# piotrprzybyszdev/Path-Tracing

Hardware: AMD Instinct MI355X
Metric: Msamples/s (paths*spp/s) at 1920x1080, 8spp, depth 8 (higher is better)
Workload: dtype f32; 1 GPU; chess_like (procedural stand-in for BASELINE configs[1] 'Khronos ABeautifulGame'), 1920x1080, 8 spp, depth 8; triangles=1999000, frames_in_flight=8, parallelism=pixel-tile shard x1, backend=wavefront, tile=32

## Files before the change

### path-tracing_amd/csrc/pt_render_host.hpp

```cpp
#pragma once

#include <type_traits>

template <typename F> static void withMode(int mode, F &&f)
{
    if (mode == 2) f(std::integral_constant<int, 2>());
    else if (mode == 1) f(std::integral_constant<int, 1>());
    else f(std::integral_constant<int, 0>());
}
template <typename F> static void withFlag(bool flag, F &&f)
{
    if (flag) f(std::true_type());
    else f(std::false_type());
}

static int ensureSlots(PtxRenderer *r, size_t slots)
{
    PathState &ps = r->paths;
    const size_t want = std::max(slots, ps.slotRad.n);
    const int mode = kernelMode(r);
    if (mode >= 1)
        HIP_TRY(r, ps.diffs.alloc(3 * want));
    if (mode == 2)
    {
// ... 55 lines not shown
    uint32_t tailBelow;
    uint32_t sortShade;
    Wavefront wf, wfAux;
};

static int counterErrors(PtxRenderer *r)
{
    const uint32_t *h = r->hostCounters;
    if (h[C_OVERFLOW])
        return fail(r, PTX_ERROR_DEVICE, "ptx_render: traversal stack overflow (tree deeper than %d levels)", kLdsStack + kGlobalSpill);
    if (h[C_OVERFLOW + 1])
        return fail(r, PTX_ERROR_DEVICE, "ptx_render: %u paths never produced a finite sample in %u attempts", h[C_OVERFLOW + 1], kMaxSampleRetries);
    return PTX_OK;
}

static int fetchCounters(PtxRenderer *r)
{
    HIP_TRY(r, hipMemcpyAsync(r->hostCounters, r->counters.p, C_COUNT * sizeof(uint32_t), hipMemcpyDeviceToHost, r->stream));
    HIP_TRY(r, hipStreamSynchronize(r->stream));
    return counterErrors(r);
}

static void launchAccumulate(PtxRenderer *r, const LaunchParams &p)
{
    k_accumulate<<<gridFor((size_t)p.slotsPerFrame * p.framesPerWave), kBlock, 0, r->stream>>>(p, r->paths.slotRad.p, accumTarget(r), nullptr, r->boundShard ? 1u : 0u);
}

static void launchTail(PtxRenderer *r, const RenderPlan &pl, int queue, uint32_t paths, BounceCtl ctl)
{
    const dim3 grid(gridFor(paths, kBlock, kMaxPersistentThreads / kBlock));
    withMode(pl.mode, [&](auto M) { k_tail<decltype(M)::value><<<grid, kBlock, 0, r->auxStream>>>(pl.p, pl.sv, pl.sc, pl.wfAux, queue, ctl); });
}

static int enqueueBounce(PtxRenderer *r, const RenderPlan &pl, uint32_t b, int qin, uint32_t est, int tail, bool fresh)
{
    hipStream_t S = r->stream, X = r->auxStream;
    PtxRenderer::BounceEvents &ev = r->bounceEvents[(b - 1) % r->bounceEvents.size()];
    const BounceCtl ctl = { b, 0u };
    const int qout = qin ^ 1, parity = (int)(b & 1u);
    k_prologue<<<1, 1, 0, S>>>(pl.wf, qin, ctl);
    HIP_TRY(r, hipEventRecord(ev.t0, S));
    withFlag(pl.mode == 2, [&](auto ALPHA) {
        const dim3 grid(traceGridFor(est, r->residentClosest[decltype(ALPHA)::value]));
        if (fresh)
            k_trace_closest<FirstBounce, decltype(ALPHA)::value><<<grid, kBlock, 0, S>>>(pl.sc, pl.wf, r->launchParams.p, pl.p.numSlots);
        else
            k_trace_closest<decltype(ALPHA)::value><<<grid, kBlock, 0, S>>>(pl.sc, pl.wf, qin, ctl);
    });
    HIP_TRY(r, hipEventRecord(ev.t1, S));
    if (b > 1)
        HIP_TRY(r, hipStreamWaitEvent(S, r->bounceEvents[(b - 2) % r->bounceEvents.size()].x2, 0));
    const uint32_t shadeGrid = gridFor((est + kShadeItems - 1) / kShadeItems);
    withFlag(pl.mode >= 1, [&](auto TEXTURED) {
        constexpr bool TEX = decltype(TEXTURED)::value;
        if (pl.sortShade && fresh)
            k_shade_sorted<FirstBounce, TEX><<<shadeGrid, kBlock, 0, S>>>(pl.p, pl.sv, pl.wf, qin, ctl);
        else if (pl.sortShade)
            k_shade_sorted<TEX><<<shadeGrid, kBlock, 0, S>>>(pl.p, pl.sv, pl.wf, qin, ctl);
        else if (fresh)
            k_shade<FirstBounce, TEX><<<shadeGrid, kBlock, 0, S>>>(pl.p, pl.sv, pl.wf, qin, ctl);
        else
            k_shade<TEX><<<shadeGrid, kBlock, 0, S>>>(pl.p, pl.sv, pl.wf, qin, ctl);
    });
    HIP_TRY(r, hipEventRecord(ev.t2, S));
    HIP_TRY(r, hipStreamWaitEvent(X, ev.t2, 0));
    HIP_TRY(r, hipEventRecord(ev.x0, X));
    withFlag(pl.mode == 2, [&](auto ALPHA) {
        k_trace_shadow<decltype(ALPHA)::value><<<traceGridFor(est, r->residentShadow[decltype(ALPHA)::value]), kBlock, 0, X>>>(pl.p, pl.sc, pl.wfAux, qout, parity);
    });
    k_apply_shadow<<<gridFor(est, kBlock, 4096u), kBlock, 0, X>>>(pl.p, pl.wfAux, parity);
    HIP_TRY(r, hipEventRecord(ev.x1, X));
    if (tail)
    {
        const uint32_t room = tail == 2 ? 4u * pl.tailBelow : pl.tailBelow;
        launchTail(r, pl, qout, est < room ? est : room, { b, tail == 2 ? 0xffffffffu : pl.tailBelow });
    }
    HIP_TRY(r, hipEventRecord(ev.x2, X));
    return PTX_OK;
}

static void hintedSchedule(const uint32_t *hint, uint32_t bounces, uint32_t tailBelow, uint32_t upperBound, std::vector<BounceStep> &steps)
{
    uint32_t last = bounces;
    if (tailBelow)
        for (uint32_t b = 1; b < bounces && b < (uint32_t)kMaxTimedBounces; b++)
            if (hint[b + 1] <= tailBelow) { last = b; break; }
    steps.clear();
    for (uint32_t b = 1; b <= last; b++)
    {
        uint32_t est = upperBound;
        if (b > 1 && b <= (uint32_t)kMaxTimedBounces)
            est = (uint32_t)std::min<uint64_t>((uint64_t)hint[b] + hint[b] / 4 + 4096, upperBound);
        steps.push_back({ b, est, (b == last && last < bounces) ? 2 : 0 });
    }
}

static int enqueueRound(PtxRenderer *r, const RenderPlan &pl, uint32_t upperBound, const uint32_t *hint, bool fresh)
{
    uint32_t last = 0;
    int qin = 0;
    if (hint)
    {
        hintedSchedule(hint, pl.bounces, pl.tailBelow, upperBound, r->hint.steps);
        for (const BounceStep &s : r->hint.steps)
        {
            if (const int rc = enqueueBounce(r, pl, s.bounce, qin, s.est, s.tail, fresh && s.bounce == 1u))
                return rc;
            last = s.bounce;
            qin ^= 1;
        }
    }
    else
    {
        uint32_t est = upperBound;
        for (uint32_t b = 1; b <= pl.bounces; b++)
        {
            if (const int rc = enqueueBounce(r, pl, b, qin, est, 0, fresh && b == 1u))
                return rc;
            last = b;
            qin ^= 1;
            if (const int rc = fetchCounters(r))
                return rc;
            est = r->hostCounters[qin ? C_ACTIVE1 : C_ACTIVE0];
            if (est == 0u)
                break;
            if (b < pl.bounces && est <= pl.tailBelow)
            {
                launchTail(r, pl, qin, est, { b, 0xffffffffu });
                HIP_TRY(r, hipEventRecord(r->bounceEvents[(b - 1) % r->bounceEvents.size()].x2, r->auxStream));
                break;
            }
        }
    }
    if (last)
        HIP_TRY(r, hipStreamWaitEvent(r->stream, r->bounceEvents[(last - 1) % r->bounceEvents.size()].x2, 0));
    HIP_TRY(r, hipGetLastError());
    return PTX_OK;
}

static int collectRender(PtxRenderer *r)
{
    if (r->pending.kind == PendingLaunch::kNone)
        return PTX_OK;
    const PendingLaunch pd = r->pending;
    r->pending = PendingLaunch();
    HIP_TRY(r, hipEventSynchronize(r->evB));
    if (const int rc = counterErrors(r))
        return rc;
    const uint32_t *h = r->hostCounters;
    r->stats.shadowRays = h[C_HITS];
// ... 5 lines not shown
    }
    unsigned long long waveSegments = 0;
    std::memcpy(&waveSegments, &h[C_WAVE_SEGMENTS], sizeof(waveSegments));
    waveSegments -= pd.deadSlots;
    r->stats.segments = waveSegments + h[C_SEGMENTS];
    r->stats.tracedRays = waveSegments;
    r->stats.retries = h[C_RETRIES];
    const uint32_t timed = pd.bounces < (uint32_t)kMaxTimedBounces ? pd.bounces : (uint32_t)kMaxTimedBounces;
    const uint32_t tailPaths = h[C_TAIL_PATHS], tailBounce = h[C_TAIL_PATHS + 1];
    for (uint32_t b = 1; b <= timed; b++)
    {
        const PtxRenderer::BounceEvents &ev = r->bounceEvents[b - 1];
        const uint32_t active = h[C_BOUNCE_ACTIVE + b];
        const bool ran = active != 0u && !(tailPaths && b > tailBounce);
        if (!ran)
            continue;
        float closestMs = 0.0f, shadeMs = 0.0f, shadowMs = 0.0f, tailMs = 0.0f;
        (void)hipEventElapsedTime(&closestMs, ev.t0, ev.t1);
        (void)hipEventElapsedTime(&shadeMs, ev.t1, ev.t2);
        (void)hipEventElapsedTime(&shadowMs, ev.x0, ev.x1);
        r->stats.lastTraceMs += closestMs;
        r->stats.lastShadeMs += shadeMs;
        r->stats.lastShadowMs += shadowMs;
        r->stats.traceLaunches += 2;
        if (tailPaths && tailBounce == b)
        {
            (void)hipEventElapsedTime(&tailMs, ev.x1, ev.x2);
            r->stats.lastTailMs += tailMs;
        }
        if (pd.verbose)
        {
            fprintf(stderr, "[ptx] bounce %u: %u rays closest %.3f ms (%.2f Grays/s) | shade (incl. wait for the previous shadow kernel) %.3f ms | shadow %.3f ms\n",
                    b, active, closestMs, active / closestMs / 1e6, shadeMs, shadowMs);
            if (tailMs > 0.0f)
                fprintf(stderr, "[ptx] tail: %u paths, %u segments, %.3f ms\n", tailPaths, h[C_SEGMENTS], tailMs);
        }
    }
    if (pd.verbose && h[C_RETRIES])
        fprintf(stderr, "[ptx] %u NaN / Inf sample restarts\n", h[C_RETRIES]);
    r->hint.active.assign(h + C_BOUNCE_ACTIVE, h + C_BOUNCE_ACTIVE + kMaxTimedBounces + 1);
    if (tailPaths && tailBounce + 1 <= (uint32_t)kMaxTimedBounces)
        r->hint.active[tailBounce + 1] = tailPaths;
    r->hint.slots = pd.slots; r->hint.bounces = pd.bounces; r->hint.epoch = pd.epoch;
    if (tailPaths > pd.tailBelow)
        r->hint.forget();
    return PTX_OK;
}

static int beginLaunch(PtxRenderer *r, const PtxLightsUbo *lights, const LaunchParams &p, uint64_t slots)
{
    HIP_TRY(r, hipSetDevice(r->device));
    if (const int rc = collectRender(r))
        return rc;
    if (const int rc = waitForCommits(r))
        return rc;
    if (slots > 0x7fffffffull)
        return fail(r, PTX_ERROR_INVALID_ARGUMENT, "ptx_render: too many path slots in one batch");
    if (const int rc = slots ? ensureSlots(r, (size_t)slots) : PTX_OK)
        return rc;
    k_upload_lights<<<1, 256, 0, r->stream>>>(*lights, p, r->lights.p, r->launchParams.p);
    HIP_TRY(r, hipMemsetAsync(r->counters.p, 0, C_COUNT * sizeof(uint32_t), r->stream));
    r->stats.pathSamples = r->stats.segments = r->stats.shadowRays = r->stats.retries = r->stats.tracedRays = 0;
    r->stats.traceLaunches = 0;
    r->stats.lastTraceMs = r->stats.lastShadeMs = r->stats.lastShadowMs = r->stats.lastTailMs = 0.0;
    HIP_TRY(r, hipEventRecord(r->evA, r->stream));
    return PTX_OK;
}

static int endLaunch(PtxRenderer *r, const PendingLaunch &pd)
{
    HIP_TRY(r, hipMemcpyAsync(r->hostCounters, r->counters.p, C_COUNT * sizeof(uint32_t), hipMemcpyDeviceToHost, r->stream));
    HIP_TRY(r, hipEventRecord(r->evB, r->stream));
    HIP_TRY(r, hipGetLastError());
// ... 43 lines not shown
    {
        if (const int rc = fetchCounters(r))
            return rc;
        const uint32_t restarts = r->hostCounters[C_RESTART];
        if (!restarts)
            return PTX_OK;
        if (round > maxRounds)
            return fail(r, PTX_ERROR_DEVICE, "ptx_render: %u paths still active after %llu rounds", restarts, (unsigned long long)maxRounds);
        k_restart<<<gridFor(restarts), kBlock, 0, r->stream>>>(pl.p, pl.wf, restarts);
        HIP_TRY(r, hipMemcpyAsync(pl.wf.queue[0], pl.wf.restartQueue, (size_t)restarts * sizeof(uint32_t), hipMemcpyDeviceToDevice, r->stream));
        HIP_TRY(r, hipMemsetAsync(&r->counters.p[C_RESTART], 0, sizeof(uint32_t), r->stream));
        HIP_TRY(r, hipMemsetD32Async(reinterpret_cast<hipDeviceptr_t>(&r->counters.p[C_ACTIVE0]), (int)restarts, 1, r->stream));
        if (const int rc = enqueueRound(r, pl, restarts, nullptr, false))
            return rc;
    }
}

static int renderWavefront(PtxRenderer *r, RenderPlan &pl, uint32_t sampleCount)
{
    const LaunchParams &p = pl.p;
    if (const int rc = ensureRenderResources(r, pl.bounces))
        return rc;
    pl.sortShade = r->env.shadeSort >= 0 ? (uint32_t)r->env.shadeSort : (sceneOf(r)->scene.mixedMaterialTypes || sceneOf(r)->scene.mixedTextured) ? 1u : 0u;
    pl.tailBelow = r->env.tailThreshold >= 0 ? (uint32_t)r->env.tailThreshold : 75000u;
    pl.wf = r->paths.view(pl.mode, r->counters.p, r->spill.p);
    pl.wfAux = r->paths.view(pl.mode, r->counters.p, r->spillAux.p);
    const bool canonical = sampleCount == 1;
    const uint64_t epoch = sceneOf(r)->sceneEpoch;
    const uint32_t *hint = canonical && r->hint.matches(p.numSlots, pl.bounces, epoch) ? r->hint.active.data() : nullptr;
    const bool fresh = r->env.firstBounce;
    if (!fresh)
        k_generate<<<gridFor(p.numSlots), kBlock, 0, r->stream>>>(p, pl.wf);
    HIP_TRY(r, hipMemsetD32Async(reinterpret_cast<hipDeviceptr_t>(&r->counters.p[C_ACTIVE0]), (int)p.numSlots, 1, r->stream));
    if (const int rc = enqueueRound(r, pl, p.numSlots, hint, fresh))
        return rc;
    if (canonical)
        finishCanonical(r, pl);
    else if (const int rc = runSampleRounds(r, pl, sampleCount))
        return rc;
    launchAccumulate(r, p);
    return endLaunch(r, { PendingLaunch::kWavefront, pl.bounces, pl.tailBelow, canonical ? p.numSlots : 0u, p.numSlots - p.ownedPixels * p.frames, epoch, r->env.verbose });
}

static int renderImpl(PtxRenderer *r, const PtxRaygenUniformData *uniform, const PtxLightsUbo *lights, uint32_t firstFrame, uint32_t frames)
{
    if (!r || !uniform || !lights)
        return fail(r, PTX_ERROR_INVALID_ARGUMENT, "ptx_render: null argument");
    if (!sceneUsable(r) || !imagePtr(r))
        return fail(r, PTX_ERROR_NOT_READY, "ptx_render: need ptx_scene_upload (or ptx_share_scene), ptx_build_accel and ptx_resize first");
    if (uniform->SampleCount == 0 || uniform->SampleCount > 0xffffu || uniform->BounceCount > 0xffffu || frames == 0)
        return fail(r, PTX_ERROR_INVALID_ARGUMENT, "ptx_render: SampleCount must be in [1, 65535], BounceCount <= 65535");
    if (lights->LightCount > PTX_MAX_LIGHT_COUNT)
        return fail(r, PTX_ERROR_INVALID_ARGUMENT, "ptx_render: LightCount %u exceeds MaxLightCount", lights->LightCount);
    RenderPlan pl;
    pl.p = makeParams(r, uniform, firstFrame, frames);
    if (const int rc = beginLaunch(r, lights, pl.p, (uint64_t)pl.p.slotsPerFrame * frames))
        return rc;
    if (pl.p.numSlots == 0)
    {
        HIP_TRY(r, hipEventRecord(r->evB, r->stream));
        return PTX_OK;
    }
    pl.sv = makeSceneView(r); pl.sc = makeTraceScene(r);
    pl.mode = kernelMode(r); pl.bounces = uniform->BounceCount;
    if (r->backend == PTX_BACKEND_MEGAKERNEL)
        return renderMegakernel(r, pl);
    if (pl.bounces == 0)
        return renderZeroBounces(r, pl.p, uniform->SampleCount);
    return renderWavefront(r, pl, uniform->SampleCount);
}

static int renderDebug(PtxRenderer *r, const PtxRaygenUniformData *uniform, const PtxLightsUbo *lights, const PtxDebugViewDesc *view)
{
    if (!r || !uniform || !lights || !view)
// ... 35 lines not shown
```

### path-tracing_amd/csrc/pt_runtime.hpp

```cpp
#pragma once

#include <algorithm>
#include <atomic>
#include <cstdarg>
#include <cstdio>
#include <cstdlib>
#include <cstring>
#include <memory>
#include <string>
#include <vector>

#include "pt_aux_kernels.hpp"
#include "pt_bvh_build.hpp"
#include "pt_debug_view.hpp"
#include "pt_denoise.hpp"
#include "pt_post.hpp"
#include "pt_present.hpp"


template <typename T> struct DevBuf
{
    T *p = nullptr;
    size_t n = 0;
    DevBuf() = default;
// ... 33 lines not shown
    uint32_t plocRadius = kPlocRadius;
    float plocShape = kPlocShape;
    bool mortonCubic = false;
    uint32_t collapse = 1;
    uint32_t reinsertPasses = 2;
    uint32_t reinsertFinal = 32;
    float splitBudget = 0.0f;
    uint32_t layout = 0;
};

struct EnvSwitches
{
    uint32_t cuPartition = 0;
    bool singleStream = false;
    bool verbose = false;
    bool karrasBuilder = false;
    bool plocFixed = false;
    uint32_t plocRadius = 0;
    float plocShape = 0.0f;
    int reinsertPasses = -1;
    float splitBudget = -1.0f;
    int layout = -1;
    int collapse = -1;
    int shadeSort = -1;
    long tailThreshold = -1;
    uint32_t framesPerWave = 8;
    uint32_t raysPerThread = 0;
    long residentCap = -1;
    uint32_t copyGroups = 0;
    bool snapshotMemcpy = false;
    bool fenceRefit = false;
    bool pairLeaves = true;
    bool firstBounce = true;
    bool streamLevelwise = false;
    static EnvSwitches read()
    {
        EnvSwitches e;
        e.verbose = getenv("PTX_VERBOSE") != nullptr;
        e.streamLevelwise = getenv("PTX_STREAM_LEVELWISE") != nullptr && std::strcmp(getenv("PTX_STREAM_LEVELWISE"), "0") != 0;
        if (const char *v = getenv("PTX_PAIR_LEAVES"))
            e.pairLeaves = std::strcmp(v, "0") != 0;
        if (const char *v = getenv("PTX_FIRST_BOUNCE"))
            e.firstBounce = std::strcmp(v, "0") != 0;
        if (const char *v = getenv("PTX_COPY_GROUPS"))
            e.copyGroups = (uint32_t)strtoul(v, nullptr, 10);
        e.snapshotMemcpy = getenv("PTX_SNAPSHOT_MEMCPY") != nullptr && std::strcmp(getenv("PTX_SNAPSHOT_MEMCPY"), "0") != 0;
        e.fenceRefit = getenv("PTX_FENCE_REFIT") != nullptr && std::strcmp(getenv("PTX_FENCE_REFIT"), "0") != 0;
        if (const char *v = getenv("PTX_BUILDER"))
            e.karrasBuilder = std::strcmp(v, "lbvh") == 0;
        if (const char *v = getenv("PTX_PLOC_SHAPE"))
        {
            e.plocFixed = true;
            e.plocShape = (float)atof(v);
        }
        if (const char *v = getenv("PTX_PLOC_RADIUS"))
        {
            e.plocFixed = true;
            e.plocRadius = std::max(1u, (uint32_t)strtoul(v, nullptr, 10));
        }
        if (const char *v = getenv("PTX_REINSERT"))
            e.reinsertPasses = atoi(v);
        if (const char *v = getenv("PTX_SPLIT_BUDGET"))
            e.splitBudget = (float)atof(v);
        if (const char *v = getenv("PTX_NODE_LAYOUT"))
            e.layout = atoi(v) ? 1 : 0;
        if (const char *v = getenv("PTX_COLLAPSE"))
            e.collapse = atoi(v) ? 1 : 0;
        if (const char *v = getenv("PTX_SHADE_SORT"))
            e.shadeSort = atoi(v) ? 1 : 0;
        if (const char *v = getenv("PTX_TAIL_THRESHOLD"))
            e.tailThreshold = (long)strtoul(v, nullptr, 10);
        if (const char *v = getenv("PTX_FRAMES_PER_WAVE"))
            e.framesPerWave = (uint32_t)atoi(v);
        if (const char *v = getenv("PTX_RAYS_PER_THREAD"))
            e.raysPerThread = std::max(1u, (uint32_t)strtoul(v, nullptr, 10));
        if (const char *v = getenv("PTX_RESIDENT_CAP"))
            e.residentCap = (long)strtoul(v, nullptr, 10);
        e.singleStream = getenv("PTX_SINGLE_STREAM") != nullptr && std::strcmp(getenv("PTX_SINGLE_STREAM"), "0") != 0;
        if (const char *v = getenv("PTX_CU_PARTITION"))
            e.cuPartition = (uint32_t)strtoul(v, nullptr, 10);
        return e;
    }
};

struct SceneData
{
    DevBuf<PtxVertex> vertices;
    DevBuf<uint32_t> indices;
    DevBuf<PtxMetallicRoughnessMaterial> mr;
    DevBuf<PtxSpecularGlossinessMaterial> sg;
    DevBuf<PtxPhongMaterial> phong;
    DevBuf<DevPair> pairs;
    DevBuf<uint32_t> pairFirst;
    DevBuf<DebugPair> debugPairs;
    DevBuf<DevTexture> renderTextures;
    DevBuf<float4> renderTexels;
    DevBuf<AlphaTex> alphaTex;
    DevBuf<uint32_t> alphaTexOf;
    DevBuf<float4> alphaQuads;
    uint32_t textureCount = 0;
    uint32_t skyKind = PTX_SKYBOX_CLEAR_COLOR;
    bool samplerNeeded = false;
// ... 15 lines not shown

struct PathState
{
    DevBuf<float4> rayO, rayD, thr, rad, hit, shD, shC, slotRad;
    DevBuf<uint32_t> hitPair, queue0, queue1, shadowQueue, restartQueue;
    DevBuf<uint8_t> shadowResult;
    DevBuf<float4> diffs;
    DevBuf<float4> decal; DevBuf<float> decalT;
    Wavefront view(int mode, uint32_t *counters, uint32_t *spill) const
    {
        Wavefront wf;
        wf.rayO = rayO.p; wf.rayD = rayD.p; wf.thr = thr.p; wf.rad = rad.p;
        wf.hit = hit.p; wf.hitPair = hitPair.p;
        wf.shD = shD.p; wf.shC = shC.p; wf.slotRad = slotRad.p;
        wf.queue[0] = queue0.p; wf.queue[1] = queue1.p; wf.shadowQueue = shadowQueue.p; wf.shadowResult = shadowResult.p;
        wf.restartQueue = restartQueue.p;
        for (int k = 0; k < 3; k++)
            wf.diff[k] = mode >= 1 ? diffs.p + (size_t)k * (diffs.n / 3) : nullptr;
        wf.decal = mode == 2 ? decal.p : nullptr;
        wf.decalT = mode == 2 ? decalT.p : nullptr;
        wf.counters = counters;
        wf.spill = spill;
        return wf;
    }
};

struct PendingLaunch
{
    enum Kind { kNone, kWavefront, kDebugView } kind = kNone;
    uint32_t bounces = 0, tailBelow = 0, slots = 0;
    uint32_t deadSlots = 0;
    uint64_t epoch = 0;
    bool verbose = false;
};

struct BounceStep { uint32_t bounce, est; int tail; };
struct ScheduleHint
{
    std::vector<uint32_t> active;
    std::vector<BounceStep> steps;
    uint32_t slots = 0, bounces = 0;
    uint64_t epoch = 0;
    bool matches(uint32_t s, uint32_t b, uint64_t e) const { return slots == s && bounces == b && epoch == e && !active.empty(); }
    void forget() { slots = 0u; }
};

struct PtxRenderer
{
    EnvSwitches env;
    int device = 0;
    uint32_t backend = PTX_BACKEND_WAVEFRONT;
    hipStream_t stream = nullptr;
    bool ownStream = false;
    bool counted = false;
    std::string error;

    SceneData scene;
    DevBuf<PtxLightsUbo> lights;
    DevBuf<LaunchParams> launchParams;
    DevBuf<AlphaTri> alphaTris;
    struct BuildState
    {
        DevBuf<Tri> triTmp;
        DevBuf<float4> boxLo, boxHi, nodeLo, nodeHi;
        DevBuf<uint32_t> sceneBounds, vals0, vals1, hist, histSums, flags;
        DevBuf<uint8_t> inert;
        DevBuf<float4> refLo, refHi;
        DevBuf<uint32_t> refTri;
        DevBuf<uint8_t> refInert;
        DevBuf<uint8_t> refPair;
        DevBuf<uint32_t> slotOf;
        bool pairRefs = false;
// ... 903 lines not shown
```

### path-tracing_amd/csrc/pt_wavefront.hpp

```cpp
#pragma once

#include <hip/hip_runtime.h>

#include "pt_bvh.hpp"

using namespace ptd;


template <typename T> struct StreamWord { typedef T type; };
template <> struct StreamWord<float4> { typedef float type __attribute__((ext_vector_type(4))); };
template <> struct StreamWord<uint4> { typedef uint32_t type __attribute__((ext_vector_type(4))); };
template <typename T> struct StreamRef
{
    T *p;
    typedef typename StreamWord<T>::type W;
    PT_DEV operator T() const
    {
        const W w = __builtin_nontemporal_load(reinterpret_cast<const W *>(p));
        T v;
        __builtin_memcpy(&v, &w, sizeof(T));
        return v;
    }
    PT_DEV void operator=(const T &v) const
    {
// ... 22 lines not shown
    Stream<float4> shC;
    Stream<float4> slotRad;
    Stream<float4> decal;
    Stream<float> decalT;
    Stream<float4> diff[3];
    uint32_t *queue[2];
    uint32_t *shadowQueue;
    uint8_t *shadowResult;
    uint32_t *restartQueue;
    uint32_t *counters;
    uint32_t *spill;
};

constexpr int kCounterStride = 32;
constexpr int kMaxTimedBounces = 64;
enum Counter
{
    C_ACTIVE0 = 0 * kCounterStride,
    C_ACTIVE1 = 1 * kCounterStride,
    C_SHADOW = 2 * kCounterStride,
    C_HITS = 3 * kCounterStride,
    C_SAMPLES = 4 * kCounterStride,
    C_RETRIES = 5 * kCounterStride,
    C_SEGMENTS = 6 * kCounterStride,
    C_OVERFLOW = 7 * kCounterStride,
    C_CHUNK = 8 * kCounterStride,
    C_CHUNK_SHADOW = 9 * kCounterStride,
    C_RESTART = 10 * kCounterStride,
    C_SHADOW1 = 11 * kCounterStride,
    C_CHUNK_SHADOW1 = 12 * kCounterStride,
    C_WAVE_SEGMENTS = 13 * kCounterStride,
    C_TAIL_PATHS = 14 * kCounterStride,
    C_BOUNCE_ACTIVE = 15 * kCounterStride,
    C_COUNT = C_BOUNCE_ACTIVE + ((kMaxTimedBounces + 1 + kCounterStride - 1) / kCounterStride) * kCounterStride
};
PT_DEV int queueCounter(int q) { return q ? (int)C_ACTIVE1 : (int)C_ACTIVE0; }
PT_DEV int shadowCounter(int parity) { return parity ? (int)C_SHADOW1 : (int)C_SHADOW; }
PT_DEV int shadowChunkCounter(int parity) { return parity ? (int)C_CHUNK_SHADOW1 : (int)C_CHUNK_SHADOW; }

struct BounceCtl
{
    uint32_t bounce;
    uint32_t tailBelow;
};
PT_DEV bool bounceRuns(const BounceCtl &c, uint32_t count) { return count != 0u && (c.bounce <= 1u || count > c.tailBelow); }

__global__ void k_prologue(Wavefront wf, int qin, BounceCtl ctl)
{
    const uint32_t count = wf.counters[queueCounter(qin)];
    const int parity = (int)(ctl.bounce & 1u);
    wf.counters[queueCounter(qin ^ 1)] = 0u;
    wf.counters[shadowCounter(parity)] = 0u;
    wf.counters[shadowChunkCounter(parity)] = 0u;
    wf.counters[C_CHUNK] = 0u;
    if (ctl.bounce <= (uint32_t)kMaxTimedBounces)
        wf.counters[C_BOUNCE_ACTIVE + ctl.bounce] = count;
    if (bounceRuns(ctl, count))
    {
        unsigned long long *seg = reinterpret_cast<unsigned long long *>(&wf.counters[C_WAVE_SEGMENTS]);
        *seg += count;
    }
}


struct LaunchParams
{
    PtxRaygenUniformData u;
// ... 330 lines not shown
        return true;
    }
    wf.slotRad[slot] = make_float4(radiance.x, radiance.y, radiance.z, 0.0f);
    return false;
}

PT_DEV void storeRestart(const Wavefront &wf, uint32_t slot, uint32_t rng, uint32_t state)
{
    wf.thr.p[slot].w = __uint_as_float(rng);
    wf.rayD.p[slot].w = __uint_as_float(state);
}
PT_DEV void loadRestart(const Wavefront &wf, uint32_t slot, uint32_t &rng, uint32_t &state)
{
    rng = __float_as_uint(wf.thr.p[slot].w);
    state = __float_as_uint(wf.rayD.p[slot].w);
}

PT_DEV void pushRestarts(const Wavefront &wf, bool restart, uint32_t slot)
{
    const uint64_t mask = __ballot(restart);
    if (!mask)
        return;
    const uint32_t lane = threadIdx.x & 63u;
    const int leader = __ffsll((unsigned long long)mask) - 1;
    uint32_t base = 0;
    if ((int)lane == leader)
        base = atomicAdd(&wf.counters[C_RESTART], (uint32_t)__popcll(mask));
    base = __shfl(base, leader);
    if (restart)
        wf.restartQueue[base + (uint32_t)__popcll(mask & ((1ull << lane) - 1ull))] = slot;
}

template <bool TEX, bool SORT, bool FIRST>
PT_DEV void shadeBody(const LaunchParams &p, const SceneView &sv, const Wavefront &wf, int qin, const BounceCtl &ctl);
template <bool TEX>
__global__ void __launch_bounds__(kBlock) k_shade(LaunchParams p, SceneView sv, Wavefront wf, int qin, BounceCtl ctl);
template <typename WHICH, bool TEX>
__global__ void __launch_bounds__(kBlock) k_shade(LaunchParams p, SceneView sv, Wavefront wf, int qin, BounceCtl ctl);
template <bool TEX>
__global__ void __launch_bounds__(kBlock) k_shade_sorted(LaunchParams p, SceneView sv, Wavefront wf, int qin, BounceCtl ctl);
template <typename WHICH, bool TEX>
__global__ void __launch_bounds__(kBlock) k_shade_sorted(LaunchParams p, SceneView sv, Wavefront wf, int qin, BounceCtl ctl);
#ifndef PT_SHADE_ATTR
#define PT_SHADE_ATTR __attribute__((amdgpu_waves_per_eu(3, 3)))
#endif
template <>
__global__ void __launch_bounds__(kBlock) PT_SHADE_ATTR k_shade<false>(LaunchParams p, SceneView sv, Wavefront wf, int qin, BounceCtl ctl)
{
    shadeBody<false, false, false>(p, sv, wf, qin, ctl);
}
template <>
__global__ void __launch_bounds__(kBlock) PT_SHADE_ATTR k_shade<FirstBounce, false>(LaunchParams p, SceneView sv, Wavefront wf, int qin, BounceCtl ctl)
{
    shadeBody<false, false, true>(p, sv, wf, qin, ctl);
}
template <>
__global__ void __launch_bounds__(kBlock) PT_SHADE_ATTR k_shade_sorted<false>(LaunchParams p, SceneView sv, Wavefront wf, int qin, BounceCtl ctl)
{
    shadeBody<false, true, false>(p, sv, wf, qin, ctl);
}
template <>
__global__ void __launch_bounds__(kBlock) PT_SHADE_ATTR k_shade_sorted<FirstBounce, false>(LaunchParams p, SceneView sv, Wavefront wf, int qin, BounceCtl ctl)
{
    shadeBody<false, true, true>(p, sv, wf, qin, ctl);
}
#ifndef PT_SHADE_TEX_ATTR
#define PT_SHADE_TEX_ATTR __attribute__((amdgpu_waves_per_eu(2, 2)))
#endif
template <>
__global__ void __launch_bounds__(kBlock) PT_SHADE_TEX_ATTR k_shade<true>(LaunchParams p, SceneView sv, Wavefront wf, int qin, BounceCtl ctl)
{
    shadeBody<true, false, false>(p, sv, wf, qin, ctl);
}
template <>
__global__ void __launch_bounds__(kBlock) PT_SHADE_TEX_ATTR k_shade<FirstBounce, true>(LaunchParams p, SceneView sv, Wavefront wf, int qin, BounceCtl ctl)
{
    shadeBody<true, false, true>(p, sv, wf, qin, ctl);
}
template <>
__global__ void __launch_bounds__(kBlock) PT_SHADE_TEX_ATTR k_shade_sorted<true>(LaunchParams p, SceneView sv, Wavefront wf, int qin, BounceCtl ctl)
{
    shadeBody<true, true, false>(p, sv, wf, qin, ctl);
}
template <>
__global__ void __launch_bounds__(kBlock) PT_SHADE_TEX_ATTR k_shade_sorted<FirstBounce, true>(LaunchParams p, SceneView sv, Wavefront wf, int qin, BounceCtl ctl)
{
    shadeBody<true, true, true>(p, sv, wf, qin, ctl);
}
template <bool TEX, bool SORT, bool FIRST>
PT_DEV void shadeBody(const LaunchParams &p, const SceneView &sv, const Wavefront &wf, int qin, const BounceCtl &ctl)
{
    __shared__ uint32_t s_cnt[2], s_base[2];
    const int qout = qin ^ 1;
    const uint32_t count = wf.counters[queueCounter(qin)];
    if (!bounceRuns(ctl, count))
        return;
    const int shadowSet = shadowCounter((int)(ctl.bounce & 1u));
    uint32_t nHits = 0, nSamples = 0, nRetries = 0;
    for (uint32_t base = blockIdx.x * blockDim.x * kShadeItems; base < count; base += gridDim.x * blockDim.x * kShadeItems)
    {
      __shared__ uint32_t s_sorted[SORT ? kBlock * kShadeItems : 1];
      constexpr uint32_t kPadSlot = 0xffffffffu;
      if (SORT)
      {
        constexpr uint32_t kKeys = 9, kWaves = kBlock / 64;
        __shared__ uint32_t s_keyCount[kWaves][kKeys], s_keyBase[kWaves][kKeys];
        const uint32_t lane = threadIdx.x & 63u, wave = threadIdx.x >> 6;
        const uint64_t lower = (1ull << lane) - 1ull;
        uint32_t mySlot[kShadeItems], myKey[kShadeItems];
        uint32_t cnt[kKeys];
        for (uint32_t k = 0; k < kKeys; k++)
            cnt[k] = 0;
        for (uint32_t item = 0; item < kShadeItems; item++)
        {
            const uint32_t i = base + item * blockDim.x + threadIdx.x;
            uint32_t sl = kPadSlot, key = kKeys - 1u;
            if (i < count)
            {
                sl = FIRST ? i : wf.queue[qin][i];
                const uint32_t pr = wf.hitPair[sl];
                if (pr == 0xffffffffu)
                    key = 0u;
                else if (pr != kDeadPair)
// ... 111 lines not shown
                    }
                }
                closestHit<TEX>(sv, F3(d4.x, d4.y, d4.z), hit.x, hit.y, hit.z, pair, __float_as_uint(hit.w), o4.w, rng, out, diff, decal);
                nHits++;

                radiance = radiance + throughput * out.Emissive;

                f3 contribution = F3s(0.0f);
                if (out.DirectLightPdf > 0.0f)
                {
                    contribution = (throughput * out.DirectLight) / out.DirectLightPdf;
                    pushShadow = !(contribution.x == 0.0f && contribution.y == 0.0f && contribution.z == 0.0f);
                }

                if (out.Pdf > 0.001f)
                    throughput = throughput * (out.Bsdf / out.Pdf);

                bool finished = false;
                const float prob = fmin_(maxComponent(throughput), 1.0f);
                uint32_t bounce = state & 0xffffu;
                if (prob < 0.001f)
                    finished = true;
                else if (prob < rnd(rng))
                    finished = true;
                else
                {
                    throughput = throughput / prob;
                    bounce = bounce + 1;
                    if (bounce >= p.u.BounceCount)
                        finished = true;
                }
                state = (state & 0xffff0000u) | bounce;

                if (pushShadow)
                {
                    const f3 sd = -normalize(out.LightDirection);
                    const uint32_t tmax = (__float_as_uint(out.LightDistance) & 0x7fffffffu) | (finished ? 0x80000000u : 0u);
                    wf.shD[slot] = make_float4(sd.x, sd.y, sd.z, __uint_as_float(tmax));
                    wf.shC[slot] = make_float4(contribution.x, contribution.y, contribution.z, __uint_as_float(state));
                }
                if (finished && !pushShadow)
                    restart = finishSample(p, wf, slot, state, radiance, nSamples, nRetries);
                else
                {
                    wf.rad[slot] = make_float4(radiance.x, radiance.y, radiance.z, 0.0f);
                    wf.rayO[slot] = make_float4(out.Position.x, out.Position.y, out.Position.z, finished ? __uint_as_float(rng) : out.MaxRoughness);
                    if (!finished)
                    {
                        wf.rayD[slot] = make_float4(out.Direction.x, out.Direction.y, out.Direction.z, __uint_as_float(state));
                        wf.thr[slot] = make_float4(throughput.x, throughput.y, throughput.z, __uint_as_float(rng));
                        if (TEX)
                            storeDiff(wf, slot, diff);
                        pushNext = true;
                    }
                }
            }
            if (restart)
                storeRestart(wf, slot, rng, state);
        }
        pushRestarts(wf, restart, slot);
        for (uint32_t k = 0; k < kShadeItems; k++)
            if (k == item)
                slots[k] = slot;
        pushBits |= (pushShadow ? 1u : 0u) << (2 * item) | (pushNext ? 2u : 0u) << (2 * item);
      }
        if (threadIdx.x < 2)
            s_cnt[threadIdx.x] = 0;
        __syncthreads();
        const uint32_t lane = threadIdx.x & 63u;
        uint32_t waveS[kShadeItems], waveN[kShadeItems];
        for (uint32_t k = 0; k < kShadeItems; k++)
        {
            const uint64_t maskS = __ballot((pushBits >> (2 * k)) & 1u), maskN = __ballot((pushBits >> (2 * k)) & 2u);
            uint32_t ws = 0, wn = 0;
            if (lane == 0)
            {
                if (maskS)
                    ws = atomicAdd(&s_cnt[0], (uint32_t)__popcll(maskS));
// ... 35 lines not shown
    PT_DEV void setEntry(uint32_t s) { staged = s; }
    PT_DEV bool load(uint32_t item, f3 &o, f3 &d, float &tmin, float &tmax)
    {
        const uint32_t slot = staged;
        const float4 o4 = wf.rayO[slot], d4 = wf.shD[slot];
        o = F3(o4.x, o4.y, o4.z);
        d = F3(d4.x, d4.y, d4.z);
        tmin = 0.00001f;
        tmax = __uint_as_float(__float_as_uint(d4.w) & 0x7fffffffu);
        finished = d4.w;
        return true;
    }
    PT_DEV void ignored(float, float, float, uint32_t, const TraceScene &) {}
    PT_DEV void improve(uint32_t, float, float, float, uint32_t) {}
    PT_DEV uint32_t bestSlot(uint32_t) const { return 0u; }
    PT_DEV void store(uint32_t item, const Hit &, bool occluded, bool) { wf.shadowResult[item] = (uint8_t)((occluded ? 0u : 1u) | (__float_as_uint(finished) >> 31 ? 2u : 0u)); }
};

template <bool ALPHA>
PT_DEV void traceShadowBody(const LaunchParams &p, const TraceScene &sc, const Wavefront &wf, int qout, int parity)
{
    const uint32_t count = wf.counters[shadowCounter(parity)];
    if (count == 0u)
        return;
    PT_DECLARE_STACK(st, kLdsStack, wf.spill)
    ShadowIO io = { wf, 0.0f, 0u };
    persistentTrace<true, ALPHA>(sc, io, count, &wf.counters[shadowChunkCounter(parity)], st);
    if (st.overflow)
        atomicAdd(&wf.counters[C_OVERFLOW], 1u);
    (void)p;
    (void)qout;
}

__global__ void __launch_bounds__(kBlock) k_apply_shadow(LaunchParams p, Wavefront wf, int parity)
{
    const uint32_t count = wf.counters[shadowCounter(parity)];
    uint32_t nSamples = 0, nRetries = 0;
    for (uint32_t base = blockIdx.x * blockDim.x; base < count; base += gridDim.x * blockDim.x)
    {
        const uint32_t item = base + threadIdx.x;
        bool restart = false;
        uint32_t slot = 0;
        if (item < count)
        {
            const uint32_t result = wf.shadowResult[item];
            slot = wf.shadowQueue[item];
            if (result)
            {
                float4 r4 = wf.rad[slot];
                const float4 c = wf.shC[slot];
                if (result & 1u)
                {
                    r4.x = r4.x + c.x;
                    r4.y = r4.y + c.y;
                    r4.z = r4.z + c.z;
                }
                if (result & 2u)
                {
                    uint32_t state = __float_as_uint(c.w);
                    f3 radiance = F3(r4.x, r4.y, r4.z);
                    restart = finishSample(p, wf, slot, state, radiance, nSamples, nRetries);
                    if (restart)
                        storeRestart(wf, slot, __float_as_uint(wf.rayO.p[slot].w), state);
                }
                else
                    wf.rad[slot] = r4;
            }
        }
        pushRestarts(wf, restart, slot);
    }
    blockAddCounter(&wf.counters[C_SAMPLES], nSamples);
    blockAddCounter(&wf.counters[C_RETRIES], nRetries);
}
template <bool ALPHA>
__global__ void __launch_bounds__(kBlock) k_trace_shadow(LaunchParams p, TraceScene sc, Wavefront wf, int qout, int parity);
template <>
__global__ void __launch_bounds__(kBlock) PT_FULL_OCCUPANCY k_trace_shadow<false>(LaunchParams p, TraceScene sc, Wavefront wf, int qout, int parity)
{
    traceShadowBody<false>(p, sc, wf, qout, parity);
}
template <>
__global__ void __launch_bounds__(kBlock) PT_ALPHA_SHADOW_ATTR k_trace_shadow<true>(LaunchParams p, TraceScene sc, Wavefront wf, int qout, int parity)
{
    traceShadowBody<true>(p, sc, wf, qout, parity);
}

__global__ void __launch_bounds__(kBlock) k_restart(LaunchParams p, Wavefront wf, uint32_t count)
{
    for (uint32_t i = blockIdx.x * blockDim.x + threadIdx.x; i < count; i += gridDim.x * blockDim.x)
    {
        const uint32_t slot = wf.restartQueue[i];
        uint32_t rng, state;
        loadRestart(wf, slot, rng, state);
        f3 o, d;
        startSlotSample(p, wf, slot, pixelOfSlot(p, slot), rng, o, d);
        wf.rayO[slot] = make_float4(o.x, o.y, o.z, 0.0f);
        wf.rayD[slot] = make_float4(d.x, d.y, d.z, __uint_as_float(state));
        wf.thr[slot] = make_float4(1.0f, 1.0f, 1.0f, __uint_as_float(rng));
    }
}

__global__ void __launch_bounds__(kBlock) k_accumulate(LaunchParams p, const float4 *__restrict__ slotRad, float4 *__restrict__ image,
                                                        const uint32_t *__restrict__ pendingRestarts, uint32_t shardMajor)
{
    if (pendingRestarts && *pendingRestarts != 0u)
// ... 468 lines not shown
```

Baseline: 2622 Msamples/s.

## Store both shadow outcomes in shade so apply_shadow touches only mismatched paths

The shade kernel now writes both the lit and unlit radiance, one to rad and the other to shC, choosing a per-bounce polarity (optimistic or pessimistic) from the visible/occluded counts of the previous launch. k_apply_shadow then reads and writes only for paths whose shadow result differs from the guessed polarity, or that finish, instead of doing a read-modify-write of rad plus a read of shC for every visible hit. This is meant to cut global memory traffic in the apply pass. It adds per-bounce counters, a host-side hint, and extra per-path stores in shade.

```diff
diff --git a/path-tracing_amd/csrc/pt_render_host.hpp b/path-tracing_amd/csrc/pt_render_host.hpp
--- a/path-tracing_amd/csrc/pt_render_host.hpp
+++ b/path-tracing_amd/csrc/pt_render_host.hpp
@@ -111,12 +111,13 @@
     withMode(pl.mode, [&](auto M) { k_tail<decltype(M)::value><<<grid, kBlock, 0, r->auxStream>>>(pl.p, pl.sv, pl.sc, pl.wfAux, queue, ctl); });
 }
 
-static int enqueueBounce(PtxRenderer *r, const RenderPlan &pl, uint32_t b, int qin, uint32_t est, int tail, bool fresh)
+static int enqueueBounce(PtxRenderer *r, const RenderPlan &pl, uint32_t b, int qin, uint32_t est, int tail, bool fresh, bool optimistic)
 {
     hipStream_t S = r->stream, X = r->auxStream;
     PtxRenderer::BounceEvents &ev = r->bounceEvents[(b - 1) % r->bounceEvents.size()];
     const BounceCtl ctl = { b, 0u };
     const int qout = qin ^ 1, parity = (int)(b & 1u);
+    const uint32_t polarity = optimistic ? 1u : 0u;
     k_prologue<<<1, 1, 0, S>>>(pl.wf, qin, ctl);
     HIP_TRY(r, hipEventRecord(ev.t0, S));
     withFlag(pl.mode == 2, [&](auto ALPHA) {
@@ -133,13 +134,13 @@
     withFlag(pl.mode >= 1, [&](auto TEXTURED) {
         constexpr bool TEX = decltype(TEXTURED)::value;
         if (pl.sortShade && fresh)
-            k_shade_sorted<FirstBounce, TEX><<<shadeGrid, kBlock, 0, S>>>(pl.p, pl.sv, pl.wf, qin, ctl);
+            k_shade_sorted<FirstBounce, TEX><<<shadeGrid, kBlock, 0, S>>>(pl.p, pl.sv, pl.wf, qin, ctl, polarity);
         else if (pl.sortShade)
-            k_shade_sorted<TEX><<<shadeGrid, kBlock, 0, S>>>(pl.p, pl.sv, pl.wf, qin, ctl);
+            k_shade_sorted<TEX><<<shadeGrid, kBlock, 0, S>>>(pl.p, pl.sv, pl.wf, qin, ctl, polarity);
         else if (fresh)
-            k_shade<FirstBounce, TEX><<<shadeGrid, kBlock, 0, S>>>(pl.p, pl.sv, pl.wf, qin, ctl);
+            k_shade<FirstBounce, TEX><<<shadeGrid, kBlock, 0, S>>>(pl.p, pl.sv, pl.wf, qin, ctl, polarity);
         else
-            k_shade<TEX><<<shadeGrid, kBlock, 0, S>>>(pl.p, pl.sv, pl.wf, qin, ctl);
+            k_shade<TEX><<<shadeGrid, kBlock, 0, S>>>(pl.p, pl.sv, pl.wf, qin, ctl, polarity);
     });
     HIP_TRY(r, hipEventRecord(ev.t2, S));
     HIP_TRY(r, hipStreamWaitEvent(X, ev.t2, 0));
@@ -147,7 +148,7 @@
     withFlag(pl.mode == 2, [&](auto ALPHA) {
         k_trace_shadow<decltype(ALPHA)::value><<<traceGridFor(est, r->residentShadow[decltype(ALPHA)::value]), kBlock, 0, X>>>(pl.p, pl.sc, pl.wfAux, qout, parity);
     });
-    k_apply_shadow<<<gridFor(est, kBlock, 4096u), kBlock, 0, X>>>(pl.p, pl.wfAux, parity);
+    k_apply_shadow<<<gridFor(est, kBlock, 4096u), kBlock, 0, X>>>(pl.p, pl.wfAux, parity, b, polarity);
     HIP_TRY(r, hipEventRecord(ev.x1, X));
     if (tail)
     {
@@ -174,16 +175,24 @@
     }
 }
 
-static int enqueueRound(PtxRenderer *r, const RenderPlan &pl, uint32_t upperBound, const uint32_t *hint, bool fresh)
+static int enqueueRound(PtxRenderer *r, const RenderPlan &pl, uint32_t upperBound, const uint32_t *hint, bool fresh, uint64_t *pessimistic = nullptr)
 {
     uint32_t last = 0;
     int qin = 0;
+    const int forced = r->env.shadowPolarity;
+    auto polarityOf = [&](uint32_t b) {
+        const bool optimistic = forced >= 0 ? forced != 0 : hint ? r->hint.optimistic(b) : true;
+        static_assert(kMaxTimedBounces <= 64, "one bit per timed bounce");
+        if (pessimistic && !optimistic && b <= (uint32_t)kMaxTimedBounces)
+            *pessimistic |= 1ull << (b - 1u);
+        return optimistic;
+    };
     if (hint)
     {
         hintedSchedule(hint, pl.bounces, pl.tailBelow, upperBound, r->hint.steps);
         for (const BounceStep &s : r->hint.steps)
         {
-            if (const int rc = enqueueBounce(r, pl, s.bounce, qin, s.est, s.tail, fresh && s.bounce == 1u))
+            if (const int rc = enqueueBounce(r, pl, s.bounce, qin, s.est, s.tail, fresh && s.bounce == 1u, polarityOf(s.bounce)))
                 return rc;
             last = s.bounce;
             qin ^= 1;
@@ -194,7 +203,7 @@
         uint32_t est = upperBound;
         for (uint32_t b = 1; b <= pl.bounces; b++)
         {
-            if (const int rc = enqueueBounce(r, pl, b, qin, est, 0, fresh && b == 1u))
+            if (const int rc = enqueueBounce(r, pl, b, qin, est, 0, fresh && b == 1u, polarityOf(b)))
                 return rc;
             last = b;
             qin ^= 1;
@@ -266,6 +275,8 @@
         {
             fprintf(stderr, "[ptx] bounce %u: %u rays closest %.3f ms (%.2f Grays/s) | shade (incl. wait for the previous shadow kernel) %.3f ms | shadow %.3f ms\n",
                     b, active, closestMs, active / closestMs / 1e6, shadeMs, shadowMs);
+            fprintf(stderr, "[ptx] bounce %u: shadow polarity %s | continuing paths: %u visible, %u occluded\n", b,
+                    (pd.pessimistic >> (b - 1u)) & 1ull ? "pessimistic" : "optimistic", h[C_SHADOW_VISIBLE + b], h[C_SHADOW_OCCLUDED + b]);
             if (tailMs > 0.0f)
                 fprintf(stderr, "[ptx] tail: %u paths, %u segments, %.3f ms\n", tailPaths, h[C_SEGMENTS], tailMs);
         }
@@ -273,6 +284,8 @@
     if (pd.verbose && h[C_RETRIES])
         fprintf(stderr, "[ptx] %u NaN / Inf sample restarts\n", h[C_RETRIES]);
     r->hint.active.assign(h + C_BOUNCE_ACTIVE, h + C_BOUNCE_ACTIVE + kMaxTimedBounces + 1);
+    r->hint.visible.assign(h + C_SHADOW_VISIBLE, h + C_SHADOW_VISIBLE + kMaxTimedBounces + 1);
+    r->hint.occluded.assign(h + C_SHADOW_OCCLUDED, h + C_SHADOW_OCCLUDED + kMaxTimedBounces + 1);
     if (tailPaths && tailBounce + 1 <= (uint32_t)kMaxTimedBounces)
         r->hint.active[tailBounce + 1] = tailPaths;
     r->hint.slots = pd.slots; r->hint.bounces = pd.bounces; r->hint.epoch = pd.epoch;
@@ -382,14 +395,15 @@
     if (!fresh)
         k_generate<<<gridFor(p.numSlots), kBlock, 0, r->stream>>>(p, pl.wf);
     HIP_TRY(r, hipMemsetD32Async(reinterpret_cast<hipDeviceptr_t>(&r->counters.p[C_ACTIVE0]), (int)p.numSlots, 1, r->stream));
-    if (const int rc = enqueueRound(r, pl, p.numSlots, hint, fresh))
+    uint64_t pessimistic = 0;
+    if (const int rc = enqueueRound(r, pl, p.numSlots, hint, fresh, &pessimistic))
         return rc;
     if (canonical)
         finishCanonical(r, pl);
     else if (const int rc = runSampleRounds(r, pl, sampleCount))
         return rc;
     launchAccumulate(r, p);
-    return endLaunch(r, { PendingLaunch::kWavefront, pl.bounces, pl.tailBelow, canonical ? p.numSlots : 0u, p.numSlots - p.ownedPixels * p.frames, epoch, r->env.verbose });
+    return endLaunch(r, { PendingLaunch::kWavefront, pl.bounces, pl.tailBelow, canonical ? p.numSlots : 0u, p.numSlots - p.ownedPixels * p.frames, epoch, r->env.verbose, pessimistic });
 }
 
 static int renderImpl(PtxRenderer *r, const PtxRaygenUniformData *uniform, const PtxLightsUbo *lights, uint32_t firstFrame, uint32_t frames)
diff --git a/path-tracing_amd/csrc/pt_runtime.hpp b/path-tracing_amd/csrc/pt_runtime.hpp
--- a/path-tracing_amd/csrc/pt_runtime.hpp
+++ b/path-tracing_amd/csrc/pt_runtime.hpp
@@ -89,6 +89,7 @@
     bool fenceRefit = false;
     bool pairLeaves = true;
     bool firstBounce = true;
+    int shadowPolarity = -1;
     bool streamLevelwise = false;
     static EnvSwitches read()
     {
@@ -125,6 +126,8 @@
             e.collapse = atoi(v) ? 1 : 0;
         if (const char *v = getenv("PTX_SHADE_SORT"))
             e.shadeSort = atoi(v) ? 1 : 0;
+        if (const char *v = getenv("PTX_SHADOW_POLARITY"))
+            e.shadowPolarity = std::strcmp(v, "0") == 0 ? 0 : std::strcmp(v, "1") == 0 ? 1 : -1;
         if (const char *v = getenv("PTX_TAIL_THRESHOLD"))
             e.tailThreshold = (long)strtoul(v, nullptr, 10);
         if (const char *v = getenv("PTX_FRAMES_PER_WAVE"))
@@ -206,12 +209,15 @@
     uint32_t deadSlots = 0;
     uint64_t epoch = 0;
     bool verbose = false;
+    uint64_t pessimistic = 0;
 };
 
 struct BounceStep { uint32_t bounce, est; int tail; };
 struct ScheduleHint
 {
     std::vector<uint32_t> active;
+    std::vector<uint32_t> visible, occluded;
+    bool optimistic(uint32_t b) const { return b >= visible.size() || b >= occluded.size() || visible[b] >= occluded[b]; }
     std::vector<BounceStep> steps;
     uint32_t slots = 0, bounces = 0;
     uint64_t epoch = 0;
diff --git a/path-tracing_amd/csrc/pt_wavefront.hpp b/path-tracing_amd/csrc/pt_wavefront.hpp
--- a/path-tracing_amd/csrc/pt_wavefront.hpp
+++ b/path-tracing_amd/csrc/pt_wavefront.hpp
@@ -78,7 +78,10 @@
     C_WAVE_SEGMENTS = 13 * kCounterStride,
     C_TAIL_PATHS = 14 * kCounterStride,
     C_BOUNCE_ACTIVE = 15 * kCounterStride,
-    C_COUNT = C_BOUNCE_ACTIVE + ((kMaxTimedBounces + 1 + kCounterStride - 1) / kCounterStride) * kCounterStride
+    kPerBounceWords = ((kMaxTimedBounces + 1 + kCounterStride - 1) / kCounterStride) * kCounterStride,
+    C_SHADOW_VISIBLE = C_BOUNCE_ACTIVE + kPerBounceWords,
+    C_SHADOW_OCCLUDED = C_SHADOW_VISIBLE + kPerBounceWords,
+    C_COUNT = C_SHADOW_OCCLUDED + kPerBounceWords
 };
 PT_DEV int queueCounter(int q) { return q ? (int)C_ACTIVE1 : (int)C_ACTIVE0; }
 PT_DEV int shadowCounter(int parity) { return parity ? (int)C_SHADOW1 : (int)C_SHADOW; }
@@ -475,63 +478,63 @@
 }
 
 template <bool TEX, bool SORT, bool FIRST>
-PT_DEV void shadeBody(const LaunchParams &p, const SceneView &sv, const Wavefront &wf, int qin, const BounceCtl &ctl);
+PT_DEV void shadeBody(const LaunchParams &p, const SceneView &sv, const Wavefront &wf, int qin, const BounceCtl &ctl, uint32_t optimistic);
 template <bool TEX>
-__global__ void __launch_bounds__(kBlock) k_shade(LaunchParams p, SceneView sv, Wavefront wf, int qin, BounceCtl ctl);
+__global__ void __launch_bounds__(kBlock) k_shade(LaunchParams p, SceneView sv, Wavefront wf, int qin, BounceCtl ctl, uint32_t optimistic);
 template <typename WHICH, bool TEX>
-__global__ void __launch_bounds__(kBlock) k_shade(LaunchParams p, SceneView sv, Wavefront wf, int qin, BounceCtl ctl);
+__global__ void __launch_bounds__(kBlock) k_shade(LaunchParams p, SceneView sv, Wavefront wf, int qin, BounceCtl ctl, uint32_t optimistic);
 template <bool TEX>
-__global__ void __launch_bounds__(kBlock) k_shade_sorted(LaunchParams p, SceneView sv, Wavefront wf, int qin, BounceCtl ctl);
+__global__ void __launch_bounds__(kBlock) k_shade_sorted(LaunchParams p, SceneView sv, Wavefront wf, int qin, BounceCtl ctl, uint32_t optimistic);
 template <typename WHICH, bool TEX>
-__global__ void __launch_bounds__(kBlock) k_shade_sorted(LaunchParams p, SceneView sv, Wavefront wf, int qin, BounceCtl ctl);
+__global__ void __launch_bounds__(kBlock) k_shade_sorted(LaunchParams p, SceneView sv, Wavefront wf, int qin, BounceCtl ctl, uint32_t optimistic);
 #ifndef PT_SHADE_ATTR
 #define PT_SHADE_ATTR __attribute__((amdgpu_waves_per_eu(3, 3)))
 #endif
 template <>
-__global__ void __launch_bounds__(kBlock) PT_SHADE_ATTR k_shade<false>(LaunchParams p, SceneView sv, Wavefront wf, int qin, BounceCtl ctl)
-{
-    shadeBody<false, false, false>(p, sv, wf, qin, ctl);
-}
-template <>
-__global__ void __launch_bounds__(kBlock) PT_SHADE_ATTR k_shade<FirstBounce, false>(LaunchParams p, SceneView sv, Wavefront wf, int qin, BounceCtl ctl)
-{
-    shadeBody<false, false, true>(p, sv, wf, qin, ctl);
-}
-template <>
-__global__ void __launch_bounds__(kBlock) PT_SHADE_ATTR k_shade_sorted<false>(LaunchParams p, SceneView sv, Wavefront wf, int qin, BounceCtl ctl)
-{
-    shadeBody<false, true, false>(p, sv, wf, qin, ctl);
-}
-template <>
-__global__ void __launch_bounds__(kBlock) PT_SHADE_ATTR k_shade_sorted<FirstBounce, false>(LaunchParams p, SceneView sv, Wavefront wf, int qin, BounceCtl ctl)
-{
-    shadeBody<false, true, true>(p, sv, wf, qin, ctl);
+__global__ void __launch_bounds__(kBlock) PT_SHADE_ATTR k_shade<false>(LaunchParams p, SceneView sv, Wavefront wf, int qin, BounceCtl ctl, uint32_t optimistic)
+{
+    shadeBody<false, false, false>(p, sv, wf, qin, ctl, optimistic);
+}
+template <>
+__global__ void __launch_bounds__(kBlock) PT_SHADE_ATTR k_shade<FirstBounce, false>(LaunchParams p, SceneView sv, Wavefront wf, int qin, BounceCtl ctl, uint32_t optimistic)
+{
+    shadeBody<false, false, true>(p, sv, wf, qin, ctl, optimistic);
+}
+template <>
+__global__ void __launch_bounds__(kBlock) PT_SHADE_ATTR k_shade_sorted<false>(LaunchParams p, SceneView sv, Wavefront wf, int qin, BounceCtl ctl, uint32_t optimistic)
+{
+    shadeBody<false, true, false>(p, sv, wf, qin, ctl, optimistic);
+}
+template <>
+__global__ void __launch_bounds__(kBlock) PT_SHADE_ATTR k_shade_sorted<FirstBounce, false>(LaunchParams p, SceneView sv, Wavefront wf, int qin, BounceCtl ctl, uint32_t optimistic)
+{
+    shadeBody<false, true, true>(p, sv, wf, qin, ctl, optimistic);
 }
 #ifndef PT_SHADE_TEX_ATTR
 #define PT_SHADE_TEX_ATTR __attribute__((amdgpu_waves_per_eu(2, 2)))
 #endif
 template <>
-__global__ void __launch_bounds__(kBlock) PT_SHADE_TEX_ATTR k_shade<true>(LaunchParams p, SceneView sv, Wavefront wf, int qin, BounceCtl ctl)
-{
-    shadeBody<true, false, false>(p, sv, wf, qin, ctl);
-}
-template <>
-__global__ void __launch_bounds__(kBlock) PT_SHADE_TEX_ATTR k_shade<FirstBounce, true>(LaunchParams p, SceneView sv, Wavefront wf, int qin, BounceCtl ctl)
-{
-    shadeBody<true, false, true>(p, sv, wf, qin, ctl);
-}
-template <>
-__global__ void __launch_bounds__(kBlock) PT_SHADE_TEX_ATTR k_shade_sorted<true>(LaunchParams p, SceneView sv, Wavefront wf, int qin, BounceCtl ctl)
-{
-    shadeBody<true, true, false>(p, sv, wf, qin, ctl);
-}
-template <>
-__global__ void __launch_bounds__(kBlock) PT_SHADE_TEX_ATTR k_shade_sorted<FirstBounce, true>(LaunchParams p, SceneView sv, Wavefront wf, int qin, BounceCtl ctl)
-{
-    shadeBody<true, true, true>(p, sv, wf, qin, ctl);
+__global__ void __launch_bounds__(kBlock) PT_SHADE_TEX_ATTR k_shade<true>(LaunchParams p, SceneView sv, Wavefront wf, int qin, BounceCtl ctl, uint32_t optimistic)
+{
+    shadeBody<true, false, false>(p, sv, wf, qin, ctl, optimistic);
+}
+template <>
+__global__ void __launch_bounds__(kBlock) PT_SHADE_TEX_ATTR k_shade<FirstBounce, true>(LaunchParams p, SceneView sv, Wavefront wf, int qin, BounceCtl ctl, uint32_t optimistic)
+{
+    shadeBody<true, false, true>(p, sv, wf, qin, ctl, optimistic);
+}
+template <>
+__global__ void __launch_bounds__(kBlock) PT_SHADE_TEX_ATTR k_shade_sorted<true>(LaunchParams p, SceneView sv, Wavefront wf, int qin, BounceCtl ctl, uint32_t optimistic)
+{
+    shadeBody<true, true, false>(p, sv, wf, qin, ctl, optimistic);
+}
+template <>
+__global__ void __launch_bounds__(kBlock) PT_SHADE_TEX_ATTR k_shade_sorted<FirstBounce, true>(LaunchParams p, SceneView sv, Wavefront wf, int qin, BounceCtl ctl, uint32_t optimistic)
+{
+    shadeBody<true, true, true>(p, sv, wf, qin, ctl, optimistic);
 }
 template <bool TEX, bool SORT, bool FIRST>
-PT_DEV void shadeBody(const LaunchParams &p, const SceneView &sv, const Wavefront &wf, int qin, const BounceCtl &ctl)
+PT_DEV void shadeBody(const LaunchParams &p, const SceneView &sv, const Wavefront &wf, int qin, const BounceCtl &ctl, uint32_t optimistic)
 {
     __shared__ uint32_t s_cnt[2], s_base[2];
     const int qout = qin ^ 1;
@@ -709,18 +712,23 @@
                 }
                 state = (state & 0xffff0000u) | bounce;
 
+                uint32_t radWord = 0u;
                 if (pushShadow)
                 {
                     const f3 sd = -normalize(out.LightDirection);
                     const uint32_t tmax = (__float_as_uint(out.LightDistance) & 0x7fffffffu) | (finished ? 0x80000000u : 0u);
                     wf.shD[slot] = make_float4(sd.x, sd.y, sd.z, __uint_as_float(tmax));
-                    wf.shC[slot] = make_float4(contribution.x, contribution.y, contribution.z, __uint_as_float(state));
+                    const float litX = radiance.x + contribution.x, litY = radiance.y + contribution.y, litZ = radiance.z + contribution.z;
+                    const bool opt = optimistic != 0u;
+                    wf.shC[slot] = make_float4(opt ? radiance.x : litX, opt ? radiance.y : litY, opt ? radiance.z : litZ, __uint_as_float(state));
+                    radiance = F3(opt ? litX : radiance.x, opt ? litY : radiance.y, opt ? litZ : radiance.z);
+                    radWord = finished ? state : 0u;
                 }
                 if (finished && !pushShadow)
                     restart = finishSample(p, wf, slot, state, radiance, nSamples, nRetries);
                 else
                 {
-                    wf.rad[slot] = make_float4(radiance.x, radiance.y, radiance.z, 0.0f);
+                    wf.rad[slot] = make_float4(radiance.x, radiance.y, radiance.z, __uint_as_float(radWord));
                     wf.rayO[slot] = make_float4(out.Position.x, out.Position.y, out.Position.z, finished ? __uint_as_float(rng) : out.MaxRoughness);
                     if (!finished)
                     {
@@ -822,10 +830,10 @@
     (void)qout;
 }
 
-__global__ void __launch_bounds__(kBlock) k_apply_shadow(LaunchParams p, Wavefront wf, int parity)
+__global__ void __launch_bounds__(kBlock) k_apply_shadow(LaunchParams p, Wavefront wf, int parity, uint32_t bounce, uint32_t optimistic)
 {
     const uint32_t count = wf.counters[shadowCounter(parity)];
-    uint32_t nSamples = 0, nRetries = 0;
+    uint32_t nSamples = 0, nRetries = 0, nVisible = 0, nOccluded = 0;
     for (uint32_t base = blockIdx.x * blockDim.x; base < count; base += gridDim.x * blockDim.x)
     {
         const uint32_t item = base + threadIdx.x;
@@ -835,32 +843,37 @@
         {
             const uint32_t result = wf.shadowResult[item];
             slot = wf.shadowQueue[item];
-            if (result)
+            const bool visible = (result & 1u) != 0u, match = visible == (optimistic != 0u);
+            if (result & 2u)
             {
-                float4 r4 = wf.rad[slot];
-                const float4 c = wf.shC[slot];
-                if (result & 1u)
+                const Stream<float4> &from = match ? wf.rad : wf.shC;
+                const float4 r4 = from[slot];
+                uint32_t state = __float_as_uint(r4.w);
+                f3 radiance = F3(r4.x, r4.y, r4.z);
+                restart = finishSample(p, wf, slot, state, radiance, nSamples, nRetries);
+                if (restart)
+                    storeRestart(wf, slot, __float_as_uint(wf.rayO.p[slot].w), state);
+            }
+            else
+            {
+                nVisible += visible ? 1u : 0u;
+                nOccluded += visible ? 0u : 1u;
+                if (!match)
                 {
-                    r4.x = r4.x + c.x;
-                    r4.y = r4.y + c.y;
-                    r4.z = r4.z + c.z;
+                    const float4 c = wf.shC[slot];
+                    wf.rad[slot] = make_float4(c.x, c.y, c.z, 0.0f);
                 }
-                if (result & 2u)
-                {
-                    uint32_t state = __float_as_uint(c.w);
-                    f3 radiance = F3(r4.x, r4.y, r4.z);
-                    restart = finishSample(p, wf, slot, state, radiance, nSamples, nRetries);
-                    if (restart)
-                        storeRestart(wf, slot, __float_as_uint(wf.rayO.p[slot].w), state);
-                }
-                else
-                    wf.rad[slot] = r4;
             }
         }
         pushRestarts(wf, restart, slot);
     }
     blockAddCounter(&wf.counters[C_SAMPLES], nSamples);
     blockAddCounter(&wf.counters[C_RETRIES], nRetries);
+    if (bounce <= (uint32_t)kMaxTimedBounces)
+    {
+        blockAddCounter(&wf.counters[C_SHADOW_VISIBLE + bounce], nVisible);
+        blockAddCounter(&wf.counters[C_SHADOW_OCCLUDED + bounce], nOccluded);
+    }
 }
 template <bool ALPHA>
 __global__ void __launch_bounds__(kBlock) k_trace_shadow(LaunchParams p, TraceScene sc, Wavefront wf, int qout, int parity);
```

After: 2615 Msamples/s. Within noise of the previous version (-0.3%).
